# WesleyHsieh0806/TAO-Amodal

Measured on AMD Instinct MI355X. Metric: box-pair IoU+match throughput, higher is better.
Workload: dtype f64

## Files before the change

tao_amodal_amd/csrc/sort.hip:

```cpp
#include <algorithm>
#include <cstdlib>
#include <cstring>

#include "common.hpp"
#include "workspace.hpp"

using namespace taoamd;

#define RS_THREADS 256
#define RS_WAVES (RS_THREADS / WAVE)
#define RS_ITEMS 8
#define RS_TILE (RS_THREADS * RS_ITEMS)
#define RS_BINS 256
#define RS_PASSES 12

struct SortBufs {
    uint64_t *key[2];
    int32_t *idx[2];
    const int32_t *cat;
    uint32_t *block_hist;
    uint32_t *digit_total;
    int32_t *skip;
    int32_t *sel;
    int64_t n;
// ... 95 lines not shown
        row[i] = run;
        run += c;
    }
}

__global__ __launch_bounds__(RS_THREADS) void rs_scatter_kernel(SortBufs b, int pass)
{
    if (b.skip[pass]) return;
    __shared__ uint32_t wave_cnt[RS_WAVES][RS_BINS];
    __shared__ uint32_t digit_base[RS_BINS];
    const int s = b.sel[pass];
    const uint64_t *__restrict__ kin = b.key[s];
    const int32_t *__restrict__ iin = b.idx[s];
    uint64_t *__restrict__ kout = b.key[s ^ 1];
    int32_t *__restrict__ iout = b.idx[s ^ 1];
    const int lane = lane_id(), wave = threadIdx.x >> 6;
    for (int i = threadIdx.x; i < RS_WAVES * RS_BINS; i += RS_THREADS)
        (&wave_cnt[0][0])[i] = 0;
    {
        uint32_t v = b.digit_total[pass * RS_BINS + threadIdx.x];
        digit_base[threadIdx.x] = v;
        __syncthreads();
        for (int off = 1; off < RS_BINS; off <<= 1) {
            uint32_t w = threadIdx.x >= off ? digit_base[threadIdx.x - off] : 0;
            __syncthreads();
            digit_base[threadIdx.x] += w;
            __syncthreads();
        }
        uint32_t incl = digit_base[threadIdx.x];
        __syncthreads();
        digit_base[threadIdx.x] = incl - v +
            b.block_hist[(int64_t)threadIdx.x * b.n_blocks + blockIdx.x];
    }
    __syncthreads();
    const int64_t base = (int64_t)blockIdx.x * RS_TILE + (int64_t)wave * (WAVE * RS_ITEMS);
    uint64_t key[RS_ITEMS];
    int32_t idx[RS_ITEMS];
    uint32_t dig[RS_ITEMS], rank[RS_ITEMS];
#pragma unroll
    for (int k = 0; k < RS_ITEMS; k++) {
        const int64_t i = base + k * WAVE + lane;
        const bool ok = i < b.n;
        key[k] = ok ? kin[i] : 0;
        idx[k] = ok ? iin[i] : 0;
        dig[k] = ok ? digit_of(pass, key[k], idx[k], b.cat) : 0xffffffffu;
    }
#pragma unroll
    for (int k = 0; k < RS_ITEMS; k++) {
        const bool ok = dig[k] != 0xffffffffu;
        uint64_t peers = __ballot(ok);
#pragma unroll
        for (int bit = 0; bit < 8; bit++) {
            const bool one = (dig[k] >> bit) & 1u;
            const uint64_t m = __ballot(one);
            peers &= one ? m : ~m;
        }
        const uint32_t below = (uint32_t)__popcll(peers & ((1ull << lane) - 1));
        uint32_t old = 0;
        if (ok) old = wave_cnt[wave][dig[k]];
        rank[k] = old + below;
        if (ok && (peers >> lane) == 1ull)
            wave_cnt[wave][dig[k]] = old + below + 1;
    }
    __syncthreads();
#pragma unroll
    for (int k = 0; k < RS_ITEMS; k++) {
        if (dig[k] == 0xffffffffu) continue;
        uint32_t off = digit_base[dig[k]] + rank[k];
        for (int w = 0; w < wave; w++) off += wave_cnt[w][dig[k]];
        kout[off] = key[k];
        iout[off] = idx[k];
    }
}

__global__ void rs_finish_kernel(SortBufs b, int32_t *__restrict__ order,
                                 int32_t *__restrict__ dst)
{
    const int s = b.sel[RS_PASSES];
    for (int64_t i = blockIdx.x * (int64_t)blockDim.x + threadIdx.x; i < b.n;
         i += (int64_t)gridDim.x * blockDim.x) {
        int32_t d = b.idx[s][i];
        if (order) order[i] = d;
        if (dst) dst[d] = (int32_t)i;
    }
}

template <class A> static void key_idx_layout(Carve &c, int64_t n, A &a)
{
    for (int i = 0; i < 2; i++) a.key[i] = c.take<uint64_t>((size_t)n);
    for (int i = 0; i < 2; i++) a.idx[i] = c.take<int32_t>((size_t)n);
}

static void rs_layout(Carve &c, int64_t n, SortBufs &b)
{
    if (n < 1) n = 1;
    b.n = n;
    b.n_blocks = (int32_t)((n + RS_TILE - 1) / RS_TILE);
    key_idx_layout(c, n, b);
    b.block_hist = c.take<uint32_t>((size_t)b.n_blocks * RS_BINS);
    b.digit_total = c.take<uint32_t>(RS_PASSES * RS_BINS);
    b.skip = c.take<int32_t>(RS_PASSES + RS_PASSES + 1);
    b.sel = Carve::at(b.skip, RS_PASSES);
}

extern "C" size_t taoamd_sort_workspace(int64_t n)
{
    SortBufs b;
    return measure([&](Carve &c) { rs_layout(c, n, b); });
}

extern "C" int taoamd_sort_by_cat_score(int64_t n, const int32_t *dt_cat,
                                        const double *dt_score, int32_t *order,
                                        int32_t *dst, void *workspace,
                                        size_t workspace_bytes, void *stream)
{
    if (n == 0) return TAOAMD_OK;
    if (n > 0x7fffffff) return TAOAMD_ERR_TOO_LARGE;
    if (!dt_cat || !workspace) return TAOAMD_ERR_ARG;
    Carve c(workspace);
    SortBufs b;
    rs_layout(c, n, b);
    if (!c.fits(workspace, workspace_bytes)) return TAOAMD_ERR_WORKSPACE;
    hipStream_t s = (hipStream_t)stream;
    b.cat = dt_cat;
    TAO_HIP(hipMemsetAsync(b.digit_total, 0, RS_PASSES * RS_BINS * 4, s));
    unsigned init_blocks = (unsigned)(b.n_blocks < 2048 ? b.n_blocks : 2048);
    TAO_TIMED("rs_init_kernel", s, rs_init_kernel<<<init_blocks, RS_THREADS, 0, s>>>(b, dt_score));
    TAO_TIMED("rs_plan_kernel", s, rs_plan_kernel<<<1, RS_BINS, 0, s>>>(b));
    for (int p = 0; p < RS_PASSES; p++) {
        TAO_TIMED("rs_hist_kernel", s, rs_hist_kernel<<<b.n_blocks, RS_THREADS, 0, s>>>(b, p));
        TAO_TIMED("rs_scan_kernel", s, rs_scan_kernel<<<RS_BINS, RS_THREADS, 0, s>>>(b, p));
        TAO_TIMED("rs_scatter_kernel", s, rs_scatter_kernel<<<b.n_blocks, RS_THREADS, 0, s>>>(b, p));
    }
    TAO_TIMED("rs_finish_kernel", s, rs_finish_kernel<<<init_blocks, 256, 0, s>>>(b, order, dst));
    TAO_LAUNCH_CHECK();
    return TAOAMD_OK;
}


#define SEG_TILE 2816
#define SEG_THREADS 256

struct SegArgs {
    const int32_t *cat_off;
    const int32_t *tile_off;
    const int32_t *cat;
    const double *score;
    uint64_t *key[2];
    int32_t *idx[2];
    int32_t *order, *dst;
    int32_t *bnd;
    int64_t n;
    int32_t n_cat, n_tiles;
};

#define SEG_RUN_MAX 64
#define SEG_LONG_MAX 8
#define SEG_ROUNDS (SEG_TILE / SEG_THREADS)

struct SegLds {
    uint64_t key[SEG_TILE];
    uint16_t pos[SEG_TILE];
    uint16_t wcnt[4][RS_BINS];
    uint32_t dbase[RS_BINS];
    uint32_t wave_tot[4];
    int32_t flag;
    int32_t n_long;
    int32_t long_s[SEG_LONG_MAX], long_e[SEG_LONG_MAX];
};

__device__ __forceinline__ void seg_passes(SegLds &L, int base, int n, int p0, int p1)
{
    const int lane = lane_id(), wave = threadIdx.x >> 6;
    const int per = ((n + 4 * WAVE - 1) / (4 * WAVE)) * WAVE;
    const int rounds = per / WAVE;
    const int w0 = wave * per;
    uint64_t kr[SEG_ROUNDS];
    uint16_t pr[SEG_ROUNDS];
#pragma unroll
    for (int r = 0; r < SEG_ROUNDS; r++) {
        const int i = w0 + r * WAVE + lane;
        const bool ok = r < rounds && i < n;
        kr[r] = ok ? L.key[base + i] : 0;
        pr[r] = ok ? L.pos[base + i] : (uint16_t)0;
    }
    __syncthreads();
#pragma nounroll
    for (int pass = p0; pass < p1; pass++) {
        for (int i = threadIdx.x; i < 4 * RS_BINS; i += SEG_THREADS)
            (&L.wcnt[0][0])[i] = 0;
        if (threadIdx.x == 0) L.flag = 0;
        __syncthreads();
        {
            const uint32_t ref = (uint32_t)(L.key[base] >> (8 * pass)) & 255u;
            bool differs = false;
#pragma unroll
            for (int r = 0; r < SEG_ROUNDS; r++)
                if (r < rounds && w0 + r * WAVE + lane < n)
                    differs |= ((uint32_t)(kr[r] >> (8 * pass)) & 255u) != ref;
            if (__ballot(differs) != 0 && lane == 0) L.flag = 2;
        }
        __syncthreads();
        if (L.flag != 2) { __syncthreads(); continue; }
        uint32_t rank[SEG_ROUNDS];
#pragma unroll
        for (int r = 0; r < SEG_ROUNDS; r++) {
            if (r < rounds) {
                const int i = w0 + r * WAVE + lane;
                const bool ok = i < n;
                const uint32_t dig = (uint32_t)(kr[r] >> (8 * pass)) & 255u;
                uint64_t peers = __ballot(ok);
#pragma unroll
                for (int bit = 0; bit < 8; bit++) {
                    const bool one = (dig >> bit) & 1u;
                    const uint64_t m = __ballot(one);
                    peers &= one ? m : ~m;
                }
                const uint32_t below = (uint32_t)__popcll(peers & ((1ull << lane) - 1));
                uint32_t old = 0;
                if (ok) old = L.wcnt[wave][dig];
                rank[r] = old + below;
                if (ok && (peers >> lane) == 1ull)
                    L.wcnt[wave][dig] = (uint16_t)(old + below + 1);
            }
        }
        __syncthreads();
        {
            const int d = threadIdx.x;
            const uint32_t c0 = L.wcnt[0][d], c1 = L.wcnt[1][d], c2 = L.wcnt[2][d],
                           c3 = L.wcnt[3][d];
            const uint32_t tot = c0 + c1 + c2 + c3;
            if (d == 0) L.flag = 0;
            uint32_t inc = tot;
#pragma unroll
            for (int off = 1; off < WAVE; off <<= 1) {
                const uint32_t v = __shfl_up(inc, off, WAVE);
                if (lane >= off) inc += v;
            }
            if (lane == WAVE - 1) L.wave_tot[wave] = inc;
            __syncthreads();
            uint32_t before = 0;
            for (int w = 0; w < wave; w++) before += L.wave_tot[w];
            const uint32_t excl = before + inc - tot;
            L.dbase[d] = excl;
            L.wcnt[0][d] = 0; L.wcnt[1][d] = (uint16_t)c0;
            L.wcnt[2][d] = (uint16_t)(c0 + c1);
            L.wcnt[3][d] = (uint16_t)(c0 + c1 + c2);
            if (tot == (uint32_t)n) L.flag = 1;
        }
        __syncthreads();
        if (L.flag) { __syncthreads(); continue; }
#pragma unroll
        for (int r = 0; r < SEG_ROUNDS; r++) {
            if (r < rounds) {
                const int i = w0 + r * WAVE + lane;
                if (i < n) {
                    const uint32_t dig = (uint32_t)(kr[r] >> (8 * pass)) & 255u;
                    const uint32_t dst = L.dbase[dig] + L.wcnt[wave][dig] + rank[r];
                    L.key[base + dst] = kr[r];
                    L.pos[base + dst] = pr[r];
                }
            }
        }
        __syncthreads();
#pragma unroll
        for (int r = 0; r < SEG_ROUNDS; r++) {
            if (r < rounds) {
                const int i = w0 + r * WAVE + lane;
                if (i < n) { kr[r] = L.key[base + i]; pr[r] = L.pos[base + i]; }
            }
        }
        __syncthreads();
    }
}

template <class Load>
__device__ __forceinline__ bool seg_sort_lds(SegLds &L, int n, Load load)
{
    bool repaired = false;
#pragma nounroll
    for (int attempt = 0; attempt < 2; attempt++) {
        load();
        if (threadIdx.x == 0) L.n_long = 0;
        __syncthreads();
        seg_passes(L, 0, n, attempt == 0 ? 4 : 0, 8);
        if (attempt == 1) break;
        if (threadIdx.x == 0) L.flag = 0;
        __syncthreads();
        {
            int state = 0;
#pragma nounroll
            for (int i = threadIdx.x + 1; i < n; i += SEG_THREADS) {
                const uint64_t prev = L.key[i - 1], cur = L.key[i];
                if ((prev >> 32) == (cur >> 32) && prev > cur) {
                    const uint32_t h = (uint32_t)(cur >> 32);
                    int s0 = i - 1, e0 = i + 1;
                    while (s0 > 0 && e0 - s0 <= SEG_RUN_MAX &&
                           (uint32_t)(L.key[s0 - 1] >> 32) == h) s0--;
                    while (e0 < n && e0 - s0 <= SEG_RUN_MAX &&
                           (uint32_t)(L.key[e0] >> 32) == h) e0++;
                    if (e0 - s0 > SEG_RUN_MAX) {
                        while (s0 > 0 && (uint32_t)(L.key[s0 - 1] >> 32) == h) s0--;
                        L.pos[s0] |= 0x4000u;
                        state = 2;
                    } else {
                        for (int j = s0; j < e0; j++) L.pos[j] |= 0x8000u;
                        state = max(state, 1);
                    }
                }
            }
            if (state) atomicMax(&L.flag, state);
        }
        __syncthreads();
        repaired = L.flag != 0;
        if (L.flag != 2) break;
#pragma nounroll
        for (int i = threadIdx.x; i < n; i += SEG_THREADS) {
            if (L.pos[i] & 0x4000u) {
                L.pos[i] &= 0xbfffu;
                const int slot = atomicAdd(&L.n_long, 1);
                if (slot < SEG_LONG_MAX) { L.long_s[slot] = i; L.long_e[slot] = n; }
            }
        }
        __syncthreads();
        const int n_long = L.n_long;
        if (n_long > SEG_LONG_MAX) { repaired = false; continue; }
        {
            for (int q = 0; q < n_long; q++) {
                const int s0 = L.long_s[q];
                const uint32_t h = (uint32_t)(L.key[s0] >> 32);
#pragma nounroll
                for (int i = s0 + 1 + threadIdx.x; i < n; i += SEG_THREADS)
                    if ((uint32_t)(L.key[i] >> 32) != h) { atomicMin(&L.long_e[q], i); break; }
            }
        }
        __syncthreads();
        for (int q = 0; q < n_long; q++)
            seg_passes(L, L.long_s[q], L.long_e[q] - L.long_s[q], 0, 4);
        break;
    }
    return repaired;
}

__device__ __forceinline__ int seg_final_slot(const SegLds &L, int i, int n, bool repaired)
{
    if (!(repaired && (L.pos[i] & 0x8000u))) return i;
    const uint64_t mine = L.key[i];
    const uint32_t h = (uint32_t)(mine >> 32);
    int s0 = i, e0 = i + 1;
    while (s0 > 0 && (uint32_t)(L.key[s0 - 1] >> 32) == h) s0--;
    while (e0 < n && (uint32_t)(L.key[e0] >> 32) == h) e0++;
    int rk = 0;
    for (int j = s0; j < e0; j++) {
        const uint64_t o = L.key[j];
        rk += (o < mine || (o == mine && j < i)) ? 1 : 0;
    }
    return s0 + rk;
}

__global__ __launch_bounds__(SEG_THREADS, 5) void seg_tile_kernel(SegArgs a)
{
    __shared__ SegLds L;
    int32_t lo = 0, hi = a.n_cat;
    while (hi - lo > 1) {
        const int32_t mid = (lo + hi) >> 1;
        if (a.tile_off[mid] <= (int32_t)blockIdx.x) lo = mid; else hi = mid;
    }
    const int32_t k = lo, t = blockIdx.x - a.tile_off[k];
    const int32_t sb = a.cat_off[k], se = a.cat_off[k + 1];
    const int32_t b = sb + t * SEG_TILE;
    const int32_t n = min(SEG_TILE, se - b);
    if (n <= 0) return;
    const int lane = lane_id(), wave = threadIdx.x >> 6;
    if (n <= WAVE) {
        if (wave != 0) return;
        const uint64_t mine = lane < n ? desc_key(a.score[b + lane]) : ~0ull;
        int rank = 0;
        for (int j = 0; j < n; j++) {
            const uint32_t lo_ = (uint32_t)__builtin_amdgcn_readlane((int)(uint32_t)mine, j);
            const uint32_t hi_ = (uint32_t)__builtin_amdgcn_readlane((int)(uint32_t)(mine >> 32), j);
            const uint64_t other = ((uint64_t)hi_ << 32) | lo_;
            rank += (other < mine || (other == mine && j < lane)) ? 1 : 0;
        }
        if (lane < n) {
            if (se - sb <= SEG_TILE) {
                if (a.order) a.order[b + rank] = b + lane;
                if (a.dst) a.dst[b + lane] = b + rank;
            } else {
                a.key[0][b + rank] = mine;
                a.idx[0][b + rank] = b + lane;
            }
        }
        return;
    }
    const bool repaired = seg_sort_lds(L, n, [&]() {
#pragma nounroll
        for (int i = threadIdx.x; i < n; i += SEG_THREADS) {
            L.key[i] = desc_key(a.score[b + i]);
            L.pos[i] = (uint16_t)i;
        }
    });
    const bool single = se - sb <= SEG_TILE;
#pragma nounroll
    for (int i = threadIdx.x; i < n; i += SEG_THREADS) {
        const uint64_t mine = L.key[i];
        const int to = seg_final_slot(L, i, n, repaired);
        const int32_t d = b + (int32_t)(L.pos[i] & 0x0fffu);
        if (single) {
            if (a.order) a.order[b + to] = d;
            if (a.dst) a.dst[d] = b + to;
        } else {
            a.key[0][b + to] = mine;
            a.idx[0][b + to] = d;
        }
    }
}

__device__ __forceinline__ int32_t rank_in(const uint64_t *__restrict__ key,
                                           const int32_t *__restrict__ idx,
                                           int32_t b, int32_t e, uint64_t k,
                                           int32_t i)
{
    int32_t lo = b, hi = e;
    while (lo < hi) {
        const int32_t mid = (lo + hi) >> 1;
        const uint64_t km = key[mid];
        const bool less = km < k || (km == k && idx[mid] < i);
        if (less) lo = mid + 1; else hi = mid;
    }
    return lo - b;
}

#ifndef SEG_KMERGE_TILES
#define SEG_KMERGE_TILES 5
#endif

__global__ __launch_bounds__(256) void seg_kmerge_kernel(SegArgs a)
{
    const int64_t p = blockIdx.x * (int64_t)blockDim.x + threadIdx.x;
    if (p >= a.n) return;
    const int32_t k = a.cat[p];
    const int32_t sb = a.cat_off[k], se = a.cat_off[k + 1];
    if (se - sb <= SEG_TILE) return;
    const uint64_t *__restrict__ kin = a.key[0];
    const int32_t *__restrict__ iin = a.idx[0];
    const uint64_t kx = kin[p];
    const int32_t ix = iin[p];
    const int32_t mine = (int32_t)((p - sb) / SEG_TILE);
    int64_t pos = sb;
    for (int32_t tb = sb, t = 0; tb < se; tb += SEG_TILE, t++) {
        const int32_t te = min(tb + SEG_TILE, se);
        pos += t == mine ? p - tb : rank_in(kin, iin, tb, te, kx, ix);
    }
    if (a.order) a.order[pos] = ix;
    if (a.dst) a.dst[ix] = (int32_t)pos;
}

#define SEG_SPLIT_TILES 32
#define SEG_BND_PER_SLOT 256

struct SegLdsX {
    SegLds L;
    int32_t idx[SEG_TILE];
    uint64_t spl_key[2 * SEG_SPLIT_TILES];
    int32_t spl_idx[2 * SEG_SPLIT_TILES];
};
struct SegLdsB {
    SegLds L;
    int32_t piece_lo[SEG_SPLIT_TILES], piece_at[SEG_SPLIT_TILES + 1];
    int32_t out_base;
};

struct SplitGeom {
    int32_t sb, n, m, s, S, q, ns, B;
    bool on;
};

__device__ __forceinline__ SplitGeom split_geom(const SegArgs &a, int32_t k)
{
    SplitGeom g;
    g.sb = a.cat_off[k];
    g.n = a.cat_off[k + 1] - g.sb;
    g.m = (g.n + SEG_TILE - 1) / SEG_TILE;
    g.on = g.m >= 2 && g.m <= SEG_SPLIT_TILES;
    g.s = g.m <= 16 ? 16 : 32;
    g.S = SEG_TILE / g.s;
    g.q = g.S - g.m;
    const int32_t last_len = g.n - (g.m - 1) * SEG_TILE;
    g.ns = (g.m - 1) * g.S + last_len / g.s;
    g.B = (g.ns + g.q - 1) / g.q;
    return g;
}

__global__ __launch_bounds__(SEG_THREADS, 3) void seg_split_kernel(SegArgs a)
{
    __shared__ SegLdsX X;
    SegLds &L = X.L;
    const SplitGeom g = split_geom(a, (int32_t)blockIdx.x);
    if (!g.on) return;
    const uint64_t *__restrict__ kin = a.key[0];
    const int32_t *__restrict__ iin = a.idx[0];
    auto src_of = [&](int i) {
        const int t = i / g.S, j = i - t * g.S;
        return g.sb + t * SEG_TILE + (j + 1) * g.s - 1;
    };
    for (int i = threadIdx.x; i < g.ns; i += SEG_THREADS) X.idx[i] = iin[src_of(i)];
    const bool repaired = seg_sort_lds(L, g.ns, [&]() {
#pragma nounroll
        for (int i = threadIdx.x; i < g.ns; i += SEG_THREADS) {
            L.key[i] = kin[src_of(i)];
            L.pos[i] = (uint16_t)i;
        }
    });
#pragma nounroll
    for (int i = threadIdx.x; i < g.ns; i += SEG_THREADS) {
        const int to = seg_final_slot(L, i, g.ns, repaired) + 1;
        if (to % g.q == 0 && to / g.q < g.B) {
            X.spl_key[to / g.q] = L.key[i];
            X.spl_idx[to / g.q] = X.idx[L.pos[i] & 0x0fffu];
        }
    }
    __syncthreads();
// ... 10 lines not shown
    __shared__ SegLdsB X;
    SegLds &L = X.L;
    int32_t lo = 0, hi = a.n_cat;
    const int32_t tile = (int32_t)(blockIdx.x >> 1);
    while (hi - lo > 1) {
        const int32_t mid = (lo + hi) >> 1;
        if (a.tile_off[mid] <= tile) lo = mid; else hi = mid;
    }
    const int32_t k = lo;
    const SplitGeom g = split_geom(a, k);
    const int32_t b = (int32_t)blockIdx.x - 2 * a.tile_off[k];
    if (!g.on || b >= g.B) return;
    const uint64_t *__restrict__ kin = a.key[0];
    const int32_t *__restrict__ iin = a.idx[0];
    const int32_t *__restrict__ bnd = a.bnd + (int64_t)(g.sb / SEG_TILE) * SEG_BND_PER_SLOT;
    if (threadIdx.x < WAVE) {
        const int t = threadIdx.x;
        int32_t plo = 0, cnt = 0;
        if (t < g.m) {
            const int32_t len_t = min(SEG_TILE, g.n - t * SEG_TILE);
            plo = b > 0 ? bnd[b * SEG_SPLIT_TILES + t] : 0;
            const int32_t phi = b + 1 < g.B ? bnd[(b + 1) * SEG_SPLIT_TILES + t] : len_t;
            cnt = phi - plo;
        }
        int32_t inc = cnt, before = plo;
#pragma unroll
        for (int off = 1; off < WAVE; off <<= 1) {
            const int32_t v = __shfl_up(inc, off, WAVE), w = __shfl_xor(before, off, WAVE);
            if ((int)threadIdx.x >= off) inc += v;
            before += w;
        }
        if (t < g.m) {
            X.piece_lo[t] = plo;
            X.piece_at[t] = inc - cnt;
        }
        if (t == g.m - 1) X.piece_at[g.m] = inc;
        if (t == 0) X.out_base = g.sb + before;
    }
    __syncthreads();
    const int32_t total = min(X.piece_at[g.m], (int32_t)SEG_TILE);
    if (total <= 0) return;
    auto src_of = [&](int i) {
        int t0 = 0, t1 = g.m;
        while (t1 - t0 > 1) {
            const int mid = (t0 + t1) >> 1;
            if (X.piece_at[mid] <= i) t0 = mid; else t1 = mid;
        }
        return g.sb + t0 * SEG_TILE + X.piece_lo[t0] + (i - X.piece_at[t0]);
    };
    const bool repaired = seg_sort_lds(L, total, [&]() {
#pragma nounroll
        for (int i = threadIdx.x; i < total; i += SEG_THREADS) {
            L.key[i] = kin[src_of(i)];
            L.pos[i] = (uint16_t)i;
        }
    });
    const int32_t out = X.out_base;
#pragma nounroll
    for (int i = threadIdx.x; i < total; i += SEG_THREADS) {
        const int32_t p = out + seg_final_slot(L, i, total, repaired);
        const int32_t d = iin[src_of((int)(L.pos[i] & 0x0fffu))];
        if (a.order) a.order[p] = d;
        if (a.dst) a.dst[d] = p;
    }
}

#define MP_PER 11

template <class KA, class KB>
__device__ __forceinline__ int32_t merge_split(KA A, int32_t na, KB B, int32_t nb, int32_t o)
{
    int32_t lo = max(0, o - nb), hi = min(o, na);
    while (lo < hi) {
        const int32_t mid = (lo + hi) >> 1;
        if (A[mid] <= B[o - mid - 1]) lo = mid + 1; else hi = mid;
    }
    return lo;
}

__global__ __launch_bounds__(256) void seg_mpass_kernel(SegArgs a, int pass, int last,
                                                        int32_t longer_than)
{
    __shared__ uint64_t m_key[SEG_TILE];
    __shared__ int32_t m_idx[SEG_TILE];
    __shared__ int32_t m_split[2];
    static_assert(256 * MP_PER == SEG_TILE, "one workgroup = one tile-sized slice");
    int32_t lo = 0, hi = a.n_cat;
    while (hi - lo > 1) {
        const int32_t mid = (lo + hi) >> 1;
        if (a.tile_off[mid] <= (int32_t)blockIdx.x) lo = mid; else hi = mid;
    }
    const int32_t k = lo;
    const int32_t sb = a.cat_off[k], se = a.cat_off[k + 1];
    if (se - sb <= longer_than) return;
    const int32_t tb = sb + ((int32_t)blockIdx.x - a.tile_off[k]) * SEG_TILE;
    const int32_t len = min(SEG_TILE, se - tb);
    if (len <= 0) return;
    const int s = pass & 1;
    const uint64_t *__restrict__ kin = a.key[s];
    const int32_t *__restrict__ iin = a.idx[s];
    const int64_t L = (int64_t)SEG_TILE << pass;
    const int64_t base = sb + ((tb - sb) / (2 * L)) * (2 * L);
    const int32_t a0 = (int32_t)base, a1 = (int32_t)min(base + L, (int64_t)se);
    const int32_t b1 = (int32_t)min((int64_t)a1 + L, (int64_t)se);
    const int32_t na = a1 - a0, nb = b1 - a1;
    const int32_t o0 = tb - a0;
    auto emit = [&](int32_t p, uint64_t kx, int32_t ix) {
        if (last) {
            if (a.order) a.order[p] = ix;
            if (a.dst) a.dst[ix] = p;
        } else {
            a.key[s ^ 1][p] = kx;
            a.idx[s ^ 1][p] = ix;
        }
    };
    if (nb <= 0) {
        for (int32_t i = threadIdx.x; i < len; i += 256) emit(tb + i, kin[tb + i], iin[tb + i]);
        return;
    }
    if (threadIdx.x == 0) m_split[0] = merge_split(kin + a0, na, kin + a1, nb, o0);
    if (threadIdx.x == 64) m_split[1] = merge_split(kin + a0, na, kin + a1, nb, o0 + len);
    __syncthreads();
    const int32_t i0 = m_split[0], i1 = m_split[1];
    const int32_t j0 = o0 - i0;
    const int32_t pa = i1 - i0, pb = len - pa;
    for (int32_t i = threadIdx.x; i < len; i += 256) {
        const int32_t src = i < pa ? a0 + i0 + i : a1 + j0 + (i - pa);
        m_key[i] = kin[src];
        m_idx[i] = iin[src];
    }
    __syncthreads();
    const int32_t q0 = min(len, (int32_t)threadIdx.x * MP_PER);
    const int32_t q1 = min(len, q0 + MP_PER);
    if (q0 >= q1) return;
    const uint64_t *A = m_key, *B = m_key + pa;
    int32_t ia = merge_split(A, pa, B, pb, q0);
    int32_t ib = q0 - ia;
    for (int32_t q = q0; q < q1; q++) {
        const bool takeA = ib >= pb || (ia < pa && A[ia] <= B[ib]);
        const int32_t from = takeA ? ia : pa + ib;
        emit(tb + q, m_key[from], m_idx[from]);
        ia += takeA ? 1 : 0;
        ib += takeA ? 0 : 1;
    }
}

static void seg_layout(Carve &c, int64_t n, SegArgs &a)
{
    if (n < 1) n = 1;
    key_idx_layout(c, n, a);
    a.bnd = c.take<int32_t>(((size_t)n / SEG_TILE + 2) * SEG_BND_PER_SLOT);
}

extern "C" size_t taoamd_sort_segments_workspace(int64_t n)
{
    SegArgs a;
    return measure([&](Carve &c) { seg_layout(c, n, a); });
}

extern "C" int taoamd_sort_segments(int64_t n, int32_t n_cat,
                                    const int32_t *cat_off,
                                    const int32_t *tile_off, int32_t n_tiles,
                                    int32_t max_segment, const int32_t *dt_cat,
                                    const double *dt_score, int32_t *order,
                                    int32_t *dst, void *workspace,
                                    size_t workspace_bytes, void *stream)
{
    if (n == 0 || n_cat == 0 || n_tiles == 0) return TAOAMD_OK;
    if (n > 0x7fffffff) return TAOAMD_ERR_TOO_LARGE;
    if (!cat_off || !tile_off || !dt_cat || !dt_score || !workspace) return TAOAMD_ERR_ARG;
    Carve c(workspace);
    SegArgs a;
    seg_layout(c, n, a);
    if (!c.fits(workspace, workspace_bytes)) return TAOAMD_ERR_WORKSPACE;
    hipStream_t s = (hipStream_t)stream;
    a.cat_off = cat_off; a.tile_off = tile_off; a.cat = dt_cat; a.score = dt_score;
    a.order = order; a.dst = dst; a.n = n; a.n_cat = n_cat; a.n_tiles = n_tiles;
    TAO_TIMED("seg_tile_kernel", s, seg_tile_kernel<<<(unsigned)n_tiles, SEG_THREADS, 0, s>>>(a));
    if (max_segment > SEG_TILE && max_segment <= (int64_t)SEG_KMERGE_TILES * SEG_TILE) {
        TAO_TIMED("seg_kmerge_kernel", s, seg_kmerge_kernel<<<(unsigned)((n + 255) / 256), 256, 0, s>>>(a));
    } else if (max_segment > SEG_TILE) {
        TAO_TIMED("seg_split_kernel", s, seg_split_kernel<<<(unsigned)n_cat, SEG_THREADS, 0, s>>>(a));
        TAO_TIMED("seg_bucket_kernel", s, seg_bucket_kernel<<<2u * (unsigned)n_tiles, SEG_THREADS, 0, s>>>(a));
        const int32_t longer_than = SEG_SPLIT_TILES * SEG_TILE;
        if (max_segment > longer_than) {
            int passes = 0;
            for (int64_t L = SEG_TILE; L < max_segment; L <<= 1) passes++;
            for (int p = 0; p < passes; p++)
                TAO_TIMED("seg_mpass_kernel", s, seg_mpass_kernel<<<(unsigned)n_tiles, 256, 0, s>>>(a, p, p == passes - 1, longer_than));
        }
    }
    TAO_LAUNCH_CHECK();
    return TAOAMD_OK;
}

#define SS_CAP 1024
#define SS_FAST 512
#ifndef SS_TARGET
#define SS_TARGET 352
#define SS_CHUNK_TILES 16
#define SS_FIRST_MERGE_PASS 4
#endif
#define SS_OVER 32
#define SS_DIRECT 1024
#define SS_CHUNK (SS_CHUNK_TILES * SEG_TILE)
#define SS_MAXB 128
#define SS_HALF_CHUNK (SS_CHUNK / 2)

struct SsChunk {
    int32_t begin, n;
    int32_t bucket0, n_buckets;
    int32_t stile0;
    int32_t final;
    int32_t cat, pad;
};

struct SsArgs {
    const double *score;
    const SsChunk *chunks;
    const int32_t *split_list, *stile_chunk, *bucket_chunk;
    int32_t *cursor;
    uint64_t *spl_key;
    int32_t *spl_idx;
    uint64_t *slot_key;
    int32_t *slot_idx;
    uint64_t *key_out;
    int32_t *idx_out;
    int32_t *order, *dst;
    int32_t *redo;
    int32_t n_buckets, n_stiles, cap_limit;
    int32_t dbg;
};
#ifdef TAOAMD_ABLATE
#define SS_DBG(a, bit) ((a).dbg & (bit))
#else
#define SS_DBG(a, bit) 0
#endif

static int g_ss_cap_limit = SS_CAP;

__host__ __device__ inline int ss_over(int32_t n) { return n > SS_HALF_CHUNK ? SS_OVER / 2 : SS_OVER; }

__device__ __forceinline__ uint32_t ss_mix(uint32_t x)
{
    x ^= x >> 16; x *= 0x7feb352du; x ^= x >> 15; x *= 0x846ca68bu; x ^= x >> 16;
    return x;
}

__device__ __forceinline__ uint64_t ss_shfl_xor64(uint64_t v, int j)
{
    const uint32_t lo = (uint32_t)__shfl_xor((int)(uint32_t)v, j, WAVE);
    const uint32_t hi = (uint32_t)__shfl_xor((int)(uint32_t)(v >> 32), j, WAVE);
    return ((uint64_t)hi << 32) | lo;
}

__device__ __forceinline__ double ss_fmin(double a, double b)
{
    double r;
    asm("v_min_f64 %0, %1, %2" : "=v"(r) : "v"(a), "v"(b));
    return r;
}
__device__ __forceinline__ double ss_fmax(double a, double b)
{
    double r;
    asm("v_max_f64 %0, %1, %2" : "=v"(r) : "v"(a), "v"(b));
    return r;
}
template <int CTRL>
__device__ __forceinline__ double ss_dpp_f64(double v)
{
    const int lo = __builtin_amdgcn_update_dpp(0, __double2loint(v), CTRL, 0xF, 0xF, true);
    const int hi = __builtin_amdgcn_update_dpp(0, __double2hiint(v), CTRL, 0xF, 0xF, true);
    return __hiloint2double(hi, lo);
}
__device__ __forceinline__ double ss_shfl_xor_f64(double v, int m)
{
#ifndef SS_NO_DPP
    switch (m) {
    case 1: return ss_dpp_f64<0xB1>(v);
    case 2: return ss_dpp_f64<0x4E>(v);
    case 3: return ss_dpp_f64<0x1B>(v);
    case 4: return ss_dpp_f64<0x1B>(ss_dpp_f64<0x141>(v));
    case 7: return ss_dpp_f64<0x141>(v);
    case 8: return ss_dpp_f64<0x128>(v);
    case 15: return ss_dpp_f64<0x140>(v);
    default: break;
    }
#endif
    const int lo = __shfl_xor(__double2loint(v), m, WAVE);
    const int hi = __shfl_xor(__double2hiint(v), m, WAVE);
    return __hiloint2double(hi, lo);
}

template <int R>
__device__ __forceinline__ void ss_bitonic_packed(double (&p)[R], int lane)
{
    constexpr int LOG_N = 6 + (R == 1 ? 0 : R == 2 ? 1 : R == 4 ? 2 : R == 8 ? 3 : R == 16 ? 4 : 5);
#pragma unroll
    for (int ls = 1; ls <= LOG_N; ls++) {
        const int size = 1 << ls;
        if (size <= R) {
#pragma unroll
            for (int r = 0; r < R; r++) {
                const int r2 = r ^ (size - 1);
                if (r < r2) {
                    const double lo = ss_fmin(p[r], p[r2]), hi = ss_fmax(p[r], p[r2]);
                    p[r] = lo;
                    p[r2] = hi;
                }
            }
        } else {
            const int m = size / R - 1;
            const bool lower = (lane & (size / R / 2)) == 0;
            if (R == 1) {
                const double o = ss_shfl_xor_f64(p[0], m);
                p[0] = ((o < p[0]) == lower) ? o : p[0];
            }
            if (R > 1) {
                constexpr int G = R / 2 < 2 ? 1 : 2;
#pragma unroll
                for (int r0 = 0; r0 < R / 2; r0 += G) {
                    double o1[G], o2[G];
#pragma unroll
                    for (int g = 0; g < G; g++) {
                        o1[g] = ss_shfl_xor_f64(p[R - 1 - (r0 + g)], m);
                        o2[g] = ss_shfl_xor_f64(p[r0 + g], m);
                    }
                    if (lower) {
#pragma unroll
                        for (int g = 0; g < G; g++) {
                            p[r0 + g] = ss_fmin(p[r0 + g], o1[g]);
// ... 294 lines not shown
    __syncthreads();
#pragma unroll
    for (int r = 0; r < SEG_ROUNDS; r++) {
        if (br[r] >= 0) {
            const int32_t at = s_base[br[r]] + rr[r];
            if (at < SS_CAP && !SS_DBG(a, 16)) {
                const int64_t s = (int64_t)(c.bucket0 + br[r]) * SS_CAP + at;
                a.slot_key[s] = kr[r];
                a.slot_idx[s] = t0 + r * SEG_THREADS + (int32_t)threadIdx.x;
            }
        }
    }
}

#define SS_KEY_BITS 35
#define SS_E_BITS 10
typedef int32_t ss_i4 __attribute__((ext_vector_type(4), aligned(4)));
typedef int32_t ss_i2 __attribute__((ext_vector_type(2), aligned(4)));

__device__ __forceinline__ int ss_shift_for(uint64_t range)
{
    const int bits = range ? 64 - __clzll((long long)range) : 0;
    return bits > SS_KEY_BITS ? bits - SS_KEY_BITS : 0;
}

template <int R>
__device__ __forceinline__ bool ss_sort_bucket(const SsArgs &a, const SsChunk &c,
                                               int32_t count, int32_t out0, int lane,
                                               const uint64_t *__restrict__ sk,
                                               const int32_t *__restrict__ si,
                                               uint64_t *__restrict__ full)
{
    static_assert(WAVE * R <= (1 << SS_E_BITS), "slot bits");
    const double pad = __longlong_as_double((long long)SS_PAD);
    uint64_t k[R];
    int32_t x[R];
    uint64_t kmin = ~0ull, kmax = 0;
    if (sk == nullptr) {
#pragma unroll
        for (int r = 0; r < R; r++) {
            const int e = r * WAVE + lane;
            k[r] = desc_key(a.score[c.begin + (e < count ? e : 0)]);
            x[r] = c.begin + e;
        }
    } else {
#pragma unroll
        for (int r = 0; r < R; r++) {
            const int e = r * WAVE + lane;
            k[r] = sk[e < count ? e : 0];
            x[r] = si[e < count ? e : 0];
        }
    }
#pragma unroll
    for (int r = 0; r < R; r++) {
        const int e = r * WAVE + lane;
        if (e < count) {
            kmin = k[r] < kmin ? k[r] : kmin;
            kmax = k[r] > kmax ? k[r] : kmax;
        } else {
            k[r] = ~0ull;
            x[r] = INT32_MAX;
        }
        full[e] = k[r];
    }
    kmin = ss_wave_min_u64(kmin);
    kmax = ss_wave_max_u64(kmax);
    const int shift = ss_shift_for(kmax - kmin);
    double p[R];
#pragma unroll
    for (int r = 0; r < R; r++) {
        const int e = r * WAVE + lane;
        p[r] = e < count
            ? __longlong_as_double((long long)((1ull << 61) |
                  (((k[r] - kmin) >> shift) << (SS_IDX_BITS + SS_E_BITS)) |
                  ((uint64_t)(x[r] - c.begin) << SS_E_BITS) | (uint64_t)e))
            : pad;
    }
    if (!SS_DBG(a, 1)) ss_bitonic_packed<R>(p, lane);
    bool bad = false;
#pragma unroll
    for (int r = 0; r < R; r++) {
        const uint64_t bits = (uint64_t)__double_as_longlong(p[r]);
        const bool ok = lane * R + r < count;
        x[r] = c.begin + (int32_t)((bits >> SS_E_BITS) & ((1u << SS_IDX_BITS) - 1));
        k[r] = ok ? full[bits & ((1u << SS_E_BITS) - 1) & (WAVE * R - 1)] : ~0ull;
        if (r > 0) bad |= k[r] < k[r - 1];
    }
    if (!SS_DBG(a, 2)) {
        const uint64_t up = ss_shfl_up64(k[R - 1]);
        bad |= lane > 0 && k[0] < up;
        if (__ballot(bad) != 0) return false;
    }
    if (lane * R + R <= count && c.final && a.order && !SS_DBG(a, 8)) {
        int32_t *o = a.order + out0 + lane * R;
        if (R == 2) *(ss_i2 *)o = ss_i2{x[0], x[1]};
#pragma unroll
        for (int q = 0; q + 4 <= R; q += 4)
            *(ss_i4 *)(o + q) = ss_i4{x[q], x[q + 1], x[q + 2], x[q + 3]};
        if (R == 1) o[0] = x[0];
    }
#pragma unroll
    for (int r = 0; r < R; r++) {
        const int e = lane * R + r;
        if (e < count) {
            const int32_t pp = out0 + e;
            if (c.final) {
                if (a.order && !SS_DBG(a, 8) && lane * R + R > count) a.order[pp] = x[r];
                if (a.dst && !SS_DBG(a, 4)) a.dst[x[r]] = pp;
            } else {
                a.key_out[pp] = k[r];
                a.idx_out[pp] = x[r];
            }
        }
    }
    return true;
}

__device__ __forceinline__ void ss_rank_bucket(const SsArgs &a, const SsChunk &c,
                                               int32_t count, int32_t out0, int lane,
                                               const uint64_t *__restrict__ sk,
                                               const int32_t *__restrict__ si)
{
    auto get = [&](int32_t e, uint64_t &k, int32_t &x) {
        if (sk == nullptr) {
            k = desc_key(a.score[c.begin + e]);
            x = c.begin + e;
        } else {
            k = sk[e];
            x = si[e];
        }
    };
    for (int32_t base = 0; base < count; base += WAVE) {
        const int32_t e = base + lane;
        uint64_t k = 0;
        int32_t x = 0, rank = 0;
        if (e < count) get(e, k, x);
        for (int32_t j = 0; j < count; j++) {
            uint64_t kj;
            int32_t xj;
            get(j, kj, xj);
            rank += (kj < k || (kj == k && xj < x)) ? 1 : 0;
        }
        if (e < count) {
            const int32_t pp = out0 + rank;
            if (c.final) {
                if (a.order) a.order[pp] = x;
                if (a.dst) a.dst[x] = pp;
            } else {
                a.key_out[pp] = k;
                a.idx_out[pp] = x;
            }
        }
    }
}

__device__ __forceinline__ bool ss_bucket_geom(const SsArgs &a, int64_t gb, int lane,
                                               SsChunk &c, int32_t &count, int32_t &before,
                                               bool &overflow)
{
    c = a.chunks[a.bucket_chunk[gb]];
    const int32_t b = (int32_t)gb - c.bucket0;
    count = c.n;
    before = 0;
    if (c.n_buckets > 1) {
        const int32_t m0 = lane < c.n_buckets ? a.cursor[c.bucket0 + lane] : 0;
        const int32_t m1 = lane + WAVE < c.n_buckets ? a.cursor[c.bucket0 + WAVE + lane] : 0;
        overflow = __ballot(m0 > a.cap_limit || m1 > a.cap_limit) != 0;
        count = b < WAVE ? __shfl(m0, b, WAVE) : __shfl(m1, b - WAVE, WAVE);
        int32_t pre = (lane < b ? m0 : 0) + (lane + WAVE < b ? m1 : 0);
#pragma unroll
        for (int off = 32; off > 0; off >>= 1) pre += __shfl_xor(pre, off, WAVE);
        before = pre;
    } else {
        overflow = count > a.cap_limit;
    }
    return !overflow;
}

__global__ __launch_bounds__(256) void ss_redo_kernel(SsArgs a)
{
    __shared__ uint64_t s_full[4][WAVE * 16];
    uint64_t *full = s_full[threadIdx.x >> 6];
    const int lane = lane_id();
    const int32_t n = a.redo[-1];
    for (int32_t i = (int32_t)blockIdx.x * 4 + (int32_t)(threadIdx.x >> 6); i < n;
         i += (int32_t)gridDim.x * 4) {
        const int64_t gb = a.redo[i];
        SsChunk c;
        int32_t count, before;
        bool overflow;
        if (!ss_bucket_geom(a, gb, lane, c, count, before, overflow) || count <= 0) continue;
        const uint64_t *sk = nullptr;
        const int32_t *si = nullptr;
        if (c.n_buckets > 1) {
            sk = a.slot_key + gb * SS_CAP;
            si = a.slot_idx + gb * SS_CAP;
        }
        const int32_t out0 = c.begin + before;
        if (count > SS_FAST && ss_sort_bucket<16>(a, c, count, out0, lane, sk, si, full)) continue;
        ss_rank_bucket(a, c, count, out0, lane, sk, si);
    }
}

__global__ __launch_bounds__(256) void ss_sort_kernel(SsArgs a)
{
    __shared__ uint64_t s_full[4][WAVE * 8];
    uint64_t *full = s_full[threadIdx.x >> 6];
    const int lane = lane_id();
    const int64_t gb = (int64_t)xcd_block(blockIdx.x, gridDim.x) * 4 + (threadIdx.x >> 6);
    if (gb >= a.n_buckets) return;
    SsChunk c;
    int32_t count, before;
    bool overflow;
    ss_bucket_geom(a, gb, lane, c, count, before, overflow);
    const int32_t b = (int32_t)gb - c.bucket0;
    if (overflow) {
        const int32_t s0 = (int32_t)((int64_t)c.n * b / c.n_buckets);
        const int32_t s1 = (int32_t)((int64_t)c.n * (b + 1) / c.n_buckets);
        for (int32_t i = s0 + lane; i < s1; i += WAVE) {
            const uint64_t ki = desc_key(a.score[c.begin + i]);
            int32_t rank = 0;
            for (int32_t j = 0; j < c.n; j++) {
                const uint64_t kj = desc_key(a.score[c.begin + j]);
                rank += (kj < ki || (kj == ki && j < i)) ? 1 : 0;
            }
            const int32_t p = c.begin + rank, d = c.begin + i;
            if (c.final) {
                if (a.order) a.order[p] = d;
                if (a.dst) a.dst[d] = p;
            } else {
                a.key_out[p] = ki;
                a.idx_out[p] = d;
            }
        }
        return;
    }
    if (count <= 0) return;
    const int32_t out0 = c.begin + before;
    const uint64_t *sk = nullptr;
    const int32_t *si = nullptr;
    if (c.n_buckets > 1) {
        sk = a.slot_key + gb * SS_CAP;
        si = a.slot_idx + gb * SS_CAP;
    }
    bool done = false;
    if (count <= 64) done = ss_sort_bucket<1>(a, c, count, out0, lane, sk, si, full);
    else if (count <= 128) done = ss_sort_bucket<2>(a, c, count, out0, lane, sk, si, full);
    else if (count <= 256) done = ss_sort_bucket<4>(a, c, count, out0, lane, sk, si, full);
    else if (count <= SS_FAST) done = ss_sort_bucket<8>(a, c, count, out0, lane, sk, si, full);
    if (!done && lane == 0) a.redo[atomicAdd(&a.redo[-1], 1)] = (int32_t)gb;
}

extern "C" int taoamd_sort_plan_host(int32_t n_cat, const int32_t *cat_off_host,
                                     int64_t *sizes, int32_t *chunks,
                                     int32_t *split_list, int32_t *stile_chunk,
                                     int32_t *bucket_chunk)
{
    if (n_cat < 0 || !cat_off_host || !sizes) return TAOAMD_ERR_ARG;
    const bool fill = chunks != nullptr;
    if (fill && (!split_list || !stile_chunk || !bucket_chunk)) return TAOAMD_ERR_ARG;
    int64_t nc = 0, ns = 0, nt = 0, nb = 0, merge = 0;
    for (int32_t k = 0; k < n_cat; k++) {
        const int64_t sb = cat_off_host[k], len = cat_off_host[k + 1] - sb;
        if (len < 0) return TAOAMD_ERR_ARG;
        if (len > SS_CHUNK) merge = 1;
        for (int64_t o = 0; o < len; o += SS_CHUNK) {
            const int32_t n = (int32_t)std::min<int64_t>(SS_CHUNK, len - o);
            const int32_t B = n <= SS_DIRECT ? 1 : (n + SS_TARGET - 1) / SS_TARGET;
            const int32_t tiles = B > 1 ? (n + SEG_TILE - 1) / SEG_TILE : 0;
            if (fill) {
                SsChunk c;
                c.begin = (int32_t)(sb + o); c.n = n; c.bucket0 = (int32_t)nb;
                c.n_buckets = B; c.stile0 = (int32_t)nt; c.final = len <= SS_CHUNK;
                c.cat = k; c.pad = 0;
                memcpy(chunks + 8 * nc, &c, sizeof c);
                if (B > 1) split_list[ns] = (int32_t)nc;
                for (int32_t t = 0; t < tiles; t++) stile_chunk[nt + t] = (int32_t)nc;
                for (int32_t b = 0; b < B; b++) bucket_chunk[nb + b] = (int32_t)nc;
            }
            nc++;
            ns += B > 1;
            nt += tiles;
            nb += B;
        }
    }
    if (nb >= INT32_MAX / 2) return TAOAMD_ERR_TOO_LARGE;
    sizes[0] = nc; sizes[1] = ns; sizes[2] = nt; sizes[3] = nb; sizes[4] = merge;
    return TAOAMD_OK;
}

static size_t ss_layout(Carve &c, int64_t n, int64_t n_buckets, int merge, SsArgs &a, SegArgs &m)
{
    if (n < 1) n = 1;
    if (n_buckets < 1) n_buckets = 1;
    const size_t nb = (size_t)n_buckets;
    const size_t cursor_ints = align256((nb + 64) * 4) / 4;
    a.cursor = c.take<int32_t>(cursor_ints + nb);
    a.redo = Carve::at(a.cursor, cursor_ints);
    a.spl_key = c.take<uint64_t>(nb);
    a.spl_idx = c.take<int32_t>(nb);
    a.slot_key = c.take<uint64_t>(nb * SS_CAP);
    a.slot_idx = c.take<int32_t>(nb * SS_CAP);
    m.key[0] = m.key[1] = nullptr; m.idx[0] = m.idx[1] = nullptr; m.bnd = nullptr;
    if (merge) key_idx_layout(c, n, m);
    return cursor_ints;
}
// ... 83 lines not shown
```

Measured before the change: 48390.

## Sort small and mid-sized category segments with single-wave kernels before tile sort

Categories whose segment length is at most SS_DIRECT are now sorted by new one-wave-per-category kernels (seg_small_kernel, seg_mid_kernel) that reuse the register bucket sort from the sample-sort path. The 256-thread tile kernel skips those categories, and it is only launched when some segment is larger than SS_DIRECT. The intent is to stop spending a full 256-thread block and its large LDS footprint on tiny segments. The cost is up to two extra launches, each with one block per category, including blocks that simply exit.

```diff
diff --git a/tao_amodal_amd/csrc/sort.hip b/tao_amodal_amd/csrc/sort.hip
--- a/tao_amodal_amd/csrc/sort.hip
+++ b/tao_amodal_amd/csrc/sort.hip
@@ -271,6 +271,7 @@
     int32_t *bnd;
     int64_t n;
     int32_t n_cat, n_tiles;
+    int32_t light;
 };
 
 #define SEG_RUN_MAX 64
@@ -487,6 +488,7 @@
     }
     const int32_t k = lo, t = blockIdx.x - a.tile_off[k];
     const int32_t sb = a.cat_off[k], se = a.cat_off[k + 1];
+    if (se - sb <= a.light) return;
     const int32_t b = sb + t * SEG_TILE;
     const int32_t n = min(SEG_TILE, se - b);
     if (n <= 0) return;
@@ -803,6 +805,8 @@
     a.bnd = c.take<int32_t>(((size_t)n / SEG_TILE + 2) * SEG_BND_PER_SLOT);
 }
 
+static void seg_sort_tiles(SegArgs &a, int32_t max_segment, hipStream_t s);
+
 extern "C" size_t taoamd_sort_segments_workspace(int64_t n)
 {
     SegArgs a;
@@ -827,7 +831,7 @@
     hipStream_t s = (hipStream_t)stream;
     a.cat_off = cat_off; a.tile_off = tile_off; a.cat = dt_cat; a.score = dt_score;
     a.order = order; a.dst = dst; a.n = n; a.n_cat = n_cat; a.n_tiles = n_tiles;
-    TAO_TIMED("seg_tile_kernel", s, seg_tile_kernel<<<(unsigned)n_tiles, SEG_THREADS, 0, s>>>(a));
+    seg_sort_tiles(a, max_segment, s);
     if (max_segment > SEG_TILE && max_segment <= (int64_t)SEG_KMERGE_TILES * SEG_TILE) {
         TAO_TIMED("seg_kmerge_kernel", s, seg_kmerge_kernel<<<(unsigned)((n + 255) / 256), 256, 0, s>>>(a));
     } else if (max_segment > SEG_TILE) {
@@ -1428,6 +1432,50 @@
             }
         }
     }
+}
+
+template <int CAP, class Sort>
+__device__ __forceinline__ void seg_light_category(const SegArgs &sa, int32_t over, Sort sort)
+{
+    __shared__ uint64_t full[CAP];
+    const int32_t k = (int32_t)blockIdx.x;
+    const int32_t sb = sa.cat_off[k], n = sa.cat_off[k + 1] - sb;
+    if (n <= over || n > CAP) return;
+    SsArgs a = {};
+    a.score = sa.score; a.order = sa.order; a.dst = sa.dst;
+    SsChunk c = {};
+    c.begin = sb; c.n = n; c.n_buckets = 1; c.final = 1;
+    const int lane = lane_id();
+    if (!sort(a, c, n, lane, full)) ss_rank_bucket(a, c, n, sb, lane, nullptr, nullptr);
+}
+
+__global__ __launch_bounds__(WAVE) void seg_small_kernel(SegArgs sa)
+{
+    seg_light_category<SS_FAST>(sa, 0, [](const SsArgs &a, const SsChunk &c, int32_t n, int lane,
+                                          uint64_t *full) {
+        if (n <= 64) return ss_sort_bucket<1>(a, c, n, c.begin, lane, nullptr, nullptr, full);
+        if (n <= 128) return ss_sort_bucket<2>(a, c, n, c.begin, lane, nullptr, nullptr, full);
+        if (n <= 256) return ss_sort_bucket<4>(a, c, n, c.begin, lane, nullptr, nullptr, full);
+        return ss_sort_bucket<8>(a, c, n, c.begin, lane, nullptr, nullptr, full);
+    });
+}
+
+__global__ __launch_bounds__(WAVE) void seg_mid_kernel(SegArgs sa)
+{
+    seg_light_category<SS_DIRECT>(sa, SS_FAST, [](const SsArgs &a, const SsChunk &c, int32_t n,
+                                                  int lane, uint64_t *full) {
+        return ss_sort_bucket<16>(a, c, n, c.begin, lane, nullptr, nullptr, full);
+    });
+}
+
+static void seg_sort_tiles(SegArgs &a, int32_t max_segment, hipStream_t s)
+{
+    a.light = SS_DIRECT;
+    TAO_TIMED("seg_small_kernel", s, seg_small_kernel<<<(unsigned)a.n_cat, WAVE, 0, s>>>(a));
+    if (max_segment > SS_FAST)
+        TAO_TIMED("seg_mid_kernel", s, seg_mid_kernel<<<(unsigned)a.n_cat, WAVE, 0, s>>>(a));
+    if (max_segment > a.light)
+        TAO_TIMED("seg_tile_kernel", s, seg_tile_kernel<<<(unsigned)a.n_tiles, SEG_THREADS, 0, s>>>(a));
 }
 
 __device__ __forceinline__ bool ss_bucket_geom(const SsArgs &a, int64_t gb, int lane,
```

Result: no change. 48410, median of 2 (+0.0%).
